# zrlhahaha/Direct12PBRRenderer

Measured on AMD Instinct MI355X. Metric: shaded Mpixel/s at 4K G-buffer (full deferred frame: clustered shade + bloom + auto-exposure + ACES), higher is better.
Workload: dtype f32

## Files before the change

direct12pbrrenderer_amd/csrc/bloom.hip:

```cpp
#include <type_traits>
#include "pbr_internal.hpp"
#include "pbr_device.hpp"

using namespace pbr;

__constant__ float c_gauss[9] = {0.0148f, 0.0459f, 0.1050f, 0.1941f, 0.2803f, 0.1941f, 0.1050f, 0.0459f, 0.0148f};

__device__ __forceinline__ float4 to4(F4 v) { return make_float4(v.x, v.y, v.z, v.w); }
__device__ __forceinline__ F4 from4(float4 v) { return f4(v.x, v.y, v.z, v.w); }

struct OutRect { int x0, y0, x1, y1, ox, oy, pitch; };
constexpr int PF_MAX_RECTS = 5;
struct OutRects {
    int n, ox, oy, pitch;
    int x0[PF_MAX_RECTS], y0[PF_MAX_RECTS], x1[PF_MAX_RECTS], y1[PF_MAX_RECTS], tiles_x[PF_MAX_RECTS], first[PF_MAX_RECTS + 1];
};
__global__ __launch_bounds__(256) void k_bloom_prefilter(const pbr_half* __restrict__ hdr, int w, int h, int pitch,
                                                           pbr_half* __restrict__ out, OutRect rc,
                                                           float tx, float ty, float threshold, float knee) {
    const int x = rc.x0 + blockIdx.x * 64 + threadIdx.x;
    const int y = rc.y0 + blockIdx.y * 4 + threadIdx.y;
    if (x >= rc.x1 || y >= rc.y1) return;
    const float u = (float)x * tx, v = (float)y * ty;
    const float ox[5] = {0.0f, -1.0f, -1.0f, 1.0f, 1.0f};
// ... 409 lines not shown
            constexpr int NR = PER_T / 2 + 2;
            const int base = (first >> 1) - 1 + (first & 1);
            V3 hrow[NR];
            const float wx0 = 1.0f - fx;
#pragma unroll
            for (int j = 0; j < NR; j++) {
                const H4* row = reinterpret_cast<const H4*>(in) + (size_t)min(base + j, ih - 1) * iw;
                const H4 c0 = row[ax0], c1 = row[ax1];
                hrow[j] = fma3(h3f(c1), fx, h3f(c0) * wx0);
            }
            auto blend = [&](auto parity) {
                constexpr int P = decltype(parity)::value;
#pragma unroll
                for (int k = 0; k < PER_T; k++) {
                    constexpr int dummy = 0; (void)dummy;
                    const int odd = (P + k) & 1;
                    const int i0 = (P + k + 1) / 2 - P;
                    const float fyk = odd ? 0.25f : 0.75f, wy0 = 1.0f - fyk;
                    const V3 r = fma3(hrow[i0 + 1], fyk, hrow[i0] * wy0);
                    smp[k] = make_float4(r.x, r.y, r.z, 0.0f);
                }
            };
            if (first & 1) blend(std::integral_constant<int, 1>{}); else blend(std::integral_constant<int, 0>{});
#pragma unroll
            for (int k = 0; k < PER_T; k++)
                if (DUAL) up[k] = reinterpret_cast<const H4*>(in2)[(size_t)(first + k) * ow + sx];
        } else {
            Tap2 taps[PER_T];
            float fy[PER_T];
#pragma unroll
            for (int k = 0; k < PER_T; k++) {
                const int jj = clampi(first + k, 0, oh - 1);
                int ay0, ay1;
                tap1d<MODE>(jj, ih, ay0, ay1, fy[k]);
                taps[k] = load_tap2<MODE>(in, iw, ax0, ax1, ay0, ay1);
                if (DUAL) up[k] = reinterpret_cast<const H4*>(in2)[(size_t)jj * ow + sx];
            }
#pragma unroll
            for (int k = 0; k < PER_T; k++) smp[k] = finish_tap2_rgb<MODE>(taps[k], fx, fy[k]);
        }
        if (has_halo) {
            const int jj = clampi(first + hk, 0, oh - 1);
            int ay0, ay1;
            tap1d<MODE>(jj, ih, ay0, ay1, hfy);
            htap = load_tap2<MODE>(in, iw, bx0, bx1, ay0, ay1);
            if (DUAL) hup = reinterpret_cast<const H4*>(in2)[(size_t)jj * ow + shx];
        }
#pragma unroll
        for (int k = 0; k < PER_T; k++) {
            line[lane] = smp[k];
            if (DUAL) line2[lane] = make_float4((float)up[k].x, (float)up[k].y, (float)up[k].z, 0.0f);
            if (has_halo && hk == k) {
                line[hc] = finish_tap2_rgb<MODE>(htap, hfx, hfy);
                if (DUAL) line2[hc] = make_float4((float)hup.x, (float)hup.y, (float)hup.z, 0.0f);
            }
            wave_sync();
            V3 g = gauss9_rgb(line + lane);
            if (DUAL) g = g + gauss9_rgb(line2 + lane);
            wave_sync();
            H4 th;
            th.x = to_half_rn(g.x); th.y = to_half_rn(g.y); th.z = to_half_rn(g.z); th.w = alpha_t;
            sT[r0 + k][lane] = th;
        }
    }
    __syncthreads();
#pragma unroll
    for (int k = 0; k < PER_O; k++) {
        const int r = wv + NW * k, y = y0 + r;
        if (x >= ow || y >= oh) continue;
        V3 a3 = v3(0.0f, 0.0f, 0.0f);
#pragma unroll
        for (int i = 0; i < 9; i++) a3 = fma3(h3f(sT[r + i][lane]), c_gauss[i], a3);
        const F4 a = f4(a3.x, a3.y, a3.z, alpha_v);
        if (TAIL == 0) {
            store_h4(out + 4 * ((size_t)y * out_pitch + x), a);
        } else {
            if (!(in_mx && y >= tr.my0 && y < tr.my1)) continue;
            const half4v a0 = round_h4(a);
            const F4 s = h4f(hdr_in[k]);
            H4 o;
            o.x = to_half_rn(s.x + (float)a0.x); o.y = to_half_rn(s.y + (float)a0.y); o.z = to_half_rn(s.z + (float)a0.z); o.w = to_half_rn(s.w + (float)a0.w);
            *reinterpret_cast<H4*>(out + 4 * ((size_t)(y - tr.by) * out_pitch + (x - tr.bx))) = o;
            if (TAIL == 2) {
                if (x >= tr.hx0 && x < tr.hx1 && y >= tr.hy0 && y < tr.hy1)
                    atomicAdd(&sh_hist[wv][luminance_bin_exact((float)o.x, (float)o.y, (float)o.z, min_log, inv_range)], 1u);
            }
        }
    }
    if (tile + (int)gridDim.x < n_tiles) __syncthreads();
    }
    if (TAIL == 2) {
        __syncthreads();
        for (int i = t; i < PBR_HISTOGRAM_BINS; i += NT) {
            uint32_t sum = 0;
#pragma unroll
            for (int w2 = 0; w2 < NW; w2++) sum += sh_hist[w2][i];
            if (sum) atomicAdd(&hist[i], sum);
        }
    }
}

__device__ __forceinline__ H4 ld_h4(const void* base, uint32_t byte_off) {
    return *reinterpret_cast<const H4*>(reinterpret_cast<const char*>(base) + byte_off);
}
__device__ __forceinline__ void gauss9_pair(const float2* e, float& ge, float& go) {
    const float s[10] = {e[0].x, e[0].y, e[1].x, e[1].y, e[2].x, e[2].y, e[3].x, e[3].y, e[4].x, e[4].y};
    float a = 0.0f, b = 0.0f;
#pragma unroll
    for (int i = 0; i < 9; i++) { a = __builtin_fmaf(s[i], c_gauss[i], a); b = __builtin_fmaf(s[i + 1], c_gauss[i], b); }
    ge = a; go = b;
}

namespace poly {
constexpr double G[9] = {0.0148, 0.0459, 0.1050, 0.1941, 0.2803, 0.1941, 0.1050, 0.0459, 0.0148};
constexpr double g(int k) { return (k < -4 || k > 4) ? 0.0 : G[k + 4]; }
constexpr float E(int j) { return (float)(0.75 * g(2 * j) + 0.25 * g(2 * j + 2) + 0.75 * g(2 * j + 1) + 0.25 * g(2 * j - 1)); }
}

template <bool DUAL, int TAIL, int TH, class VS = NoViews>
__global__ __launch_bounds__(512, 4) void k_blur_up_poly(const pbr_half* __restrict__ in_, int iw, int ih,
                                                          const pbr_half* __restrict__ in2_,
                                                          pbr_half* __restrict__ out_, int ow, int oh, int out_pitch_,
                                                          int tiles_x, int n_tiles,
                                                          TailRect tr, float min_log, float inv_range, VS vs,
                                                          uint32_t* __restrict__ hist_) {
    const pbr_half* __restrict__ in = in_;
    const pbr_half* __restrict__ in2 = in2_;
    pbr_half* __restrict__ out = out_;
    uint32_t* __restrict__ hist = hist_;
    int out_pitch = out_pitch_;
    if constexpr (!std::is_same_v<VS, NoViews>) {
        const int v = blockIdx.y;
        in = vs.in[v]; in2 = vs.in2[v]; out = vs.out[v]; hist = vs.hist[v]; out_pitch = vs.out_pitch[v];
    }
    constexpr int TW = 128, NP = TW / 2 + 4, NC = TW / 2 + 6, SR = TH + 8, NT = 512, NW = NT / 64;
    constexpr int NPAIR = TH / 2 + 5;
    constexpr int PPW = (NPAIR + NW - 1) / NW;
    constexpr int PER_O = TH / 4;
    static_assert(TH % 4 == 0 && (PPW + 1) * 6 <= 64 && 2 * PPW * 4 <= 64, "one halo entry per lane");
    __shared__ H4 sLineC[NW][NC + 2];
    __shared__ float2 sLineU[DUAL ? NW : 1][3][NP];
    __shared__ H4 sT[SR][TW];
    __shared__ uint32_t sh_hist[TAIL == 2 ? NW : 1][TAIL == 2 ? PBR_HISTOGRAM_BINS : 1];
    static_assert(sizeof(sLineC) + sizeof(sLineU) + sizeof(sT) + sizeof(sh_hist) <= 80 * 1024, "k_blur_up_poly: two blocks per CU no longer fit the LDS");
    const int t = threadIdx.x, lane = t & 63;
    const int wv = __builtin_amdgcn_readfirstlane(t >> 6);
    const int vc = t & 127, vg = __builtin_amdgcn_readfirstlane(t >> 7);
    if (TAIL == 2) {
        for (int i = t; i < NW * PBR_HISTOGRAM_BINS; i += NT) (&sh_hist[0][0])[i] = 0u;
    }
    const size_t a_at = (size_t)min(tr.my0 >> 1, ih - 1) * iw + min(tr.mx0 >> 1, iw - 1);
    float alpha_h = gauss9_const((float)reinterpret_cast<const H4*>(in)[a_at].w);
    if (DUAL) alpha_h = alpha_h + gauss9_const((float)reinterpret_cast<const H4*>(in2)[(size_t)min(tr.my0, oh - 1) * ow + min(tr.mx0, ow - 1)].w);
    const h16 alpha_t = to_half_rn(alpha_h);
    const float alpha_v = gauss9_const((float)alpha_t);
    const float a0w = (float)to_half_rn(alpha_v);
    auto wave_sync = [] {
        __builtin_amdgcn_fence(__ATOMIC_RELEASE, "wavefront");
        __builtin_amdgcn_wave_barrier();
        __builtin_amdgcn_fence(__ATOMIC_ACQUIRE, "wavefront");
    };
    for (int tile = blockIdx.x; tile < n_tiles; tile += gridDim.x) {
    const int x0 = (tr.tx0 + tile % tiles_x) * TW, y0 = (tr.ty0 + tile / tiles_x) * TH;
    const int xv = x0 + vc, rbase = vg * PER_O;
    H4 hdr_in[PER_O];
    const bool in_mx = TAIL != 0 && xv >= tr.mx0 && xv < tr.mx1;
    char* const hdr_row0 = reinterpret_cast<char*>(out) + (ptrdiff_t)(y0 + rbase - tr.by) * out_pitch * 8;
    const uint32_t hdr_x = (uint32_t)(xv - tr.bx) * 8u;
    const size_t hdr_pitch = (size_t)out_pitch * 8u;
    {
        const int i_first = wv * PPW;
        const int n_pairs = min(PPW, NPAIR - i_first);
        const int cb = (y0 >> 1) - 3 + i_first;
        const uint32_t ccol = (uint32_t)clampi((x0 >> 1) - 3 + lane, 0, iw - 1) * 8u;
        H4 cr[PPW + 1], chalo{};
        const int hk = lane / 6, hq = 64 + lane % 6;
        const bool has_halo = lane < 6 * (PPW + 1);
        H4 upE[DUAL ? 2 * PPW : 1], upO[DUAL ? 2 * PPW : 1], hupE{}, hupO{};
        const int uk = lane >> 2, uq = 64 + (lane & 3);
        const bool has_uhalo = DUAL && lane < 8 * PPW;
        if (n_pairs > 0) {
#pragma unroll
            for (int k = 0; k <= PPW; k++) {
                const char* row = reinterpret_cast<const char*>(in) + (size_t)clampi(cb + k, 0, ih - 1) * iw * 8u;
                cr[k] = ld_h4(row, ccol);
            }
            if (has_halo) {
                const char* row = reinterpret_cast<const char*>(in) + (size_t)clampi(cb + hk, 0, ih - 1) * iw * 8u;
                chalo = ld_h4(row, (uint32_t)clampi((x0 >> 1) - 3 + hq, 0, iw - 1) * 8u);
            }
            if (DUAL) {
                const int sxe = clampi(x0 - 4 + 2 * lane, 0, ow - 1), sxo = clampi(x0 - 3 + 2 * lane, 0, ow - 1);
#pragma unroll
                for (int k = 0; k < 2 * PPW; k++) {
                    const char* row = reinterpret_cast<const char*>(in2) + (size_t)clampi(y0 - 4 + 2 * i_first - 1 + k, 0, oh - 1) * ow * 8u;
                    upE[k] = ld_h4(row, (uint32_t)sxe * 8u); upO[k] = ld_h4(row, (uint32_t)sxo * 8u);
                }
                if (has_uhalo) {
                    const uint32_t row = (uint32_t)(clampi(y0 - 4 + 2 * i_first - 1 + uk, 0, oh - 1) * ow) * 8u;
                    hupE = ld_h4(in2, row + (uint32_t)clampi(x0 - 4 + 2 * uq, 0, ow - 1) * 8u); hupO = ld_h4(in2, row + (uint32_t)clampi(x0 - 3 + 2 * uq, 0, ow - 1) * 8u);
                }
            }
        }
        if (TAIL != 0) {
#pragma unroll
            for (int k = 0; k < PER_O; k++) {
                const int y = y0 + rbase + k;
                if (in_mx && y >= tr.my0 && y < tr.my1) hdr_in[k] = ld_h4(hdr_row0 + k * hdr_pitch, hdr_x);
            }
        }
        if (n_pairs > 0) {
            H4* line = sLineC[wv];
            float2 (*lineU)[NP] = sLineU[DUAL ? wv : 0];
            V3 pE = v3(0.0f, 0.0f, 0.0f), pO = pE;
#pragma unroll
            for (int k = 0; k <= PPW; k++) {
                if (k > n_pairs) break;
                line[lane] = cr[k];
                if (has_halo && hk == k) line[hq] = chalo;
                wave_sync();
                V3 e[7];
#pragma unroll
                for (int j = 0; j < 7; j++) e[j] = h3f(line[lane + j]);
                wave_sync();
                constexpr float PE[6] = {poly::E(-3), poly::E(-2), poly::E(-1), poly::E(0), poly::E(1), poly::E(2)};
                V3 cE = v3(0.0f, 0.0f, 0.0f), cO = cE;
#pragma unroll
                for (int j = 0; j < 6; j++) { cE = fma3(e[j], PE[j], cE); cO = fma3(e[j + 1], PE[5 - j], cO); }
                if (k > 0) {
#pragma unroll
                    for (int half = 0; half < 2; half++) {
                        const int r = 2 * (i_first + k - 1) - 1 + half;
                        if (r < 0 || r >= SR) continue;
                        const float fy = half ? 0.75f : 0.25f, wy0 = 1.0f - fy;
                        V3 bE = fma3(cE, fy, pE * wy0), bO = fma3(cO, fy, pO * wy0);
                        if (DUAL) {
                            const int u = 2 * (k - 1) + half;
                            lineU[0][lane] = make_float2((float)upE[u].x, (float)upO[u].x); lineU[1][lane] = make_float2((float)upE[u].y, (float)upO[u].y);
                            lineU[2][lane] = make_float2((float)upE[u].z, (float)upO[u].z);
                            if (has_uhalo && uk == u) {
                                lineU[0][uq] = make_float2((float)hupE.x, (float)hupO.x); lineU[1][uq] = make_float2((float)hupE.y, (float)hupO.y);
                                lineU[2][uq] = make_float2((float)hupE.z, (float)hupO.z);
                            }
                            wave_sync();
                            V3 uE, uO;
                            gauss9_pair(lineU[0] + lane, uE.x, uO.x); gauss9_pair(lineU[1] + lane, uE.y, uO.y); gauss9_pair(lineU[2] + lane, uE.z, uO.z);
                            wave_sync();
                            bE = bE + uE; bO = bO + uO;
                        }
                        struct alignas(16) H8 { H4 a, b; } th;
                        th.a.x = to_half_rn(bE.x); th.a.y = to_half_rn(bE.y); th.a.z = to_half_rn(bE.z); th.a.w = alpha_t;
                        th.b.x = to_half_rn(bO.x); th.b.y = to_half_rn(bO.y); th.b.z = to_half_rn(bO.z); th.b.w = alpha_t;
                        *reinterpret_cast<H8*>(&sT[r][2 * lane]) = th;
                    }
                }
                pE = cE; pO = cO;
            }
        }
    }
    __syncthreads();
    {
        H4 win[PER_O + 8];
#pragma unroll
        for (int i = 0; i < PER_O + 8; i++) win[i] = sT[rbase + i][vc];
#pragma unroll
        for (int k = 0; k < PER_O; k++) {
            const int y = y0 + rbase + k;
            if (xv >= ow || y >= oh) continue;
            V3 a3 = v3(0.0f, 0.0f, 0.0f);
#pragma unroll
            for (int i = 0; i < 9; i++) a3 = fma3(h3f(win[k + i]), c_gauss[i], a3);
            const F4 a = f4(a3.x, a3.y, a3.z, alpha_v);
            if (TAIL == 0) {
                store_h4(out + 4 * ((size_t)y * out_pitch + xv), a);
            } else {
                if (!(in_mx && y >= tr.my0 && y < tr.my1)) continue;
                const half2v a01 = round_h2(a3.x, a3.y);
                const h16 a2 = to_half_rn(a3.z);
                const F4 s = h4f(hdr_in[k]);
                struct alignas(8) O4 { half2v lo, hi; } o;
                o.lo = round_h2(s.x + (float)a01.x, s.y + (float)a01.y);
                o.hi = round_h2(s.z + (float)a2, s.w + a0w);
                *reinterpret_cast<O4*>(hdr_row0 + k * hdr_pitch + hdr_x) = o;
                if (TAIL == 2) {
                    if (xv >= tr.hx0 && xv < tr.hx1 && y >= tr.hy0 && y < tr.hy1)
                        atomicAdd(&sh_hist[wv][luminance_bin_exact((float)o.lo.x, (float)o.lo.y, (float)o.hi.x, min_log, inv_range)], 1u);
                }
            }
        }
    }
    if (tile + (int)gridDim.x < n_tiles) __syncthreads();
    }
    if (TAIL == 2) {
        __syncthreads();
        for (int i = t; i < PBR_HISTOGRAM_BINS; i += NT) {
            uint32_t sum = 0;
#pragma unroll
            for (int w2 = 0; w2 < NW; w2++) sum += sh_hist[w2][i];
            if (sum) atomicAdd(&hist[i], sum);
        }
    }
}

static int blur_h_rows(uint32_t ow, uint32_t oh) {
    const uint64_t row_blocks = (uint64_t)((ow + 255) / 256) * oh;
    int rows = (int)(row_blocks / 2048);
    return rows < 1 ? 1 : (rows > HB_MAX_ROWS ? HB_MAX_ROWS : rows);
}

static bool exact_half(uint32_t n) { return (n & 1u) == 0u && n <= 8192u; }

template <int MODE, bool DUAL, int TAIL, bool MV = false>
static pbr_status launch_hv(pbr_ctx* ctx, const LevelViews& lv, uint32_t nv, uint32_t iw, uint32_t ih, uint32_t ow, uint32_t oh,
                            const uint32_t* rect, float min_log, float inv_range,
                            const uint32_t* merge_rect = nullptr, const uint32_t* buf_origin = nullptr) {
    using VS = std::conditional_t<MV, LevelViews, NoViews>;
    VS vs{};
    if constexpr (MV) vs = lv;
    const pbr_half* in = MV ? nullptr : lv.in[0];
    const pbr_half* in2 = MV ? nullptr : lv.in2[0];
    pbr_half* out = MV ? nullptr : lv.out[0];
    uint32_t* hist = MV ? nullptr : lv.hist[0];
    const int out_pitch = MV ? 0 : lv.out_pitch[0];
    TailRect tr;
    tr.hx0 = rect ? (int)rect[0] : 0; tr.hy0 = rect ? (int)rect[1] : 0;
    tr.hx1 = rect ? (int)(rect[0] + rect[2]) : 0; tr.hy1 = rect ? (int)(rect[1] + rect[3]) : 0;
    tr.mx0 = merge_rect ? (int)merge_rect[0] : 0; tr.my0 = merge_rect ? (int)merge_rect[1] : 0;
    tr.mx1 = merge_rect ? (int)(merge_rect[0] + merge_rect[2]) : (int)ow; tr.my1 = merge_rect ? (int)(merge_rect[1] + merge_rect[3]) : (int)oh;
    tr.bx = buf_origin ? (int)buf_origin[0] : 0; tr.by = buf_origin ? (int)buf_origin[1] : 0;
    static const int hist_blocks = pbr::knob_int("PBR_BLOOM_HIST_BLOCKS", 1024);
    auto even_blocks = [nv](int n_tiles) { const int per = (n_tiles * (int)nv + hist_blocks - 1) / hist_blocks; return (n_tiles + per - 1) / per; };
    if constexpr (MODE == M_UP) {
        static const int wide_forced = pbr::knob_int("PBR_BLOOM_WIDE", -1);
        const int wtx0 = tr.mx0 / 128, wty0 = tr.my0 / 32;
        const int wtiles_x = (tr.mx1 + 127) / 128 - wtx0, wn = wtiles_x * ((tr.my1 + 31) / 32 - wty0);
        if (wide_forced >= 0 ? wide_forced == 1 : (wn >= 400 && !ctx->bloom_shader_order)) {
            tr.tx0 = wtx0; tr.ty0 = wty0;
            const int wb = TAIL == 2 ? even_blocks(wn) : wn;
            hipLaunchKernelGGL((k_blur_up_poly<DUAL, TAIL, 32, VS>), dim3(wb, nv), dim3(512), 0, ctx->stream,
                               in, (int)iw, (int)ih, in2, out, (int)ow, (int)oh, out_pitch, wtiles_x, wn, tr, min_log, inv_range, vs, hist);
            return launched(ctx, MV ? "k_blur_up_poly<views>" : "k_blur_up_poly");
        }
    }
    const bool big = (uint64_t)((tr.mx1 + 63) / 64 - tr.mx0 / 64) * ((tr.my1 + 31) / 32 - tr.my0 / 32) >= 900;
    const int th = big ? 32 : 16;
    tr.tx0 = tr.mx0 / 64; tr.ty0 = tr.my0 / th;
    const int tiles_x = (tr.mx1 + 63) / 64 - tr.tx0;
    const int n_tiles = tiles_x * ((tr.my1 + th - 1) / th - tr.ty0);
    const int blocks = TAIL == 2 ? even_blocks(n_tiles) : n_tiles;
    if (big) {
        hipLaunchKernelGGL((k_blur_hv<MODE, DUAL, TAIL, 32, 512, VS>), dim3(blocks, nv), dim3(512), 0, ctx->stream,
                           in, (int)iw, (int)ih, in2, out, (int)ow, (int)oh, out_pitch, tiles_x, n_tiles, tr, min_log, inv_range, vs, hist);
    } else {
        hipLaunchKernelGGL((k_blur_hv<MODE, DUAL, TAIL, 16, 512, VS>), dim3(blocks, nv), dim3(512), 0, ctx->stream,
                           in, (int)iw, (int)ih, in2, out, (int)ow, (int)oh, out_pitch, tiles_x, n_tiles, tr, min_log, inv_range, vs, hist);
    }
    return launched(ctx, MV ? "k_blur_hv<views>" : "k_blur_hv");
}

static OutRects out_rects(const OutRect* rcs, int n) {
    OutRects rs{};
    rs.n = n; rs.ox = rcs[0].ox; rs.oy = rcs[0].oy; rs.pitch = rcs[0].pitch;
    int blocks = 0;
    for (int r = 0; r < n; r++) {
        rs.x0[r] = rcs[r].x0; rs.y0[r] = rcs[r].y0; rs.x1[r] = rcs[r].x1; rs.y1[r] = rcs[r].y1;
        rs.tiles_x[r] = (rcs[r].x1 - rcs[r].x0 + PF_TW - 1) / PF_TW;
        rs.first[r] = blocks;
        blocks += rs.tiles_x[r] * ((rcs[r].y1 - rcs[r].y0 + PF_TH - 1) / PF_TH);
    }
    rs.first[n] = blocks;
    return rs;
}

extern "C" {

static pbr_status prefilter_launch(pbr_ctx* ctx, const pbr_half* hdr, uint32_t w, uint32_t h, uint32_t pitch,
                                   pbr_half* out, const OutRect* rcs, int n, float threshold, float knee) {
    const uint32_t ow = w >> 1, oh = h >> 1;
    const float tx = 1.0f / (float)ow, ty = 1.0f / (float)oh;
    if (exact_half(w) && exact_half(h)) {
        const OutRects rs = out_rects(rcs, n);
        hipLaunchKernelGGL(k_bloom_prefilter_2x<NoViews>, dim3(rs.first[n]), dim3(256), 0, ctx->stream, hdr, (int)w, (int)h, (int)pitch, NoViews{}, out, rs, threshold, knee);
        return launched(ctx, "k_bloom_prefilter_2x");
    }
    for (int r = 0; r < n; r++) {
        const uint32_t rw = (uint32_t)(rcs[r].x1 - rcs[r].x0), rh = (uint32_t)(rcs[r].y1 - rcs[r].y0);
        dim3 grid((rw + 63) / 64, (rh + 3) / 4);
        hipLaunchKernelGGL(k_bloom_prefilter, grid, dim3(64, 4), 0, ctx->stream, hdr, (int)w, (int)h, (int)pitch, out, rcs[r], tx, ty, threshold, knee);
        pbr_status st = launched(ctx, "k_bloom_prefilter");
        if (st) return st;
    }
    return PBR_OK;
}

pbr_status pbr_bloom_prefilter(pbr_ctx* ctx, const pbr_half* hdr, uint32_t w, uint32_t h, uint32_t pitch,
                               pbr_half* out, float threshold, float knee) {
    if (!ctx) return PBR_ERR_INVALID;
    PBR_REQUIRE(ctx, hdr && out, "pbr_bloom_prefilter: null pointer");
    PBR_REQUIRE(ctx, (w >> 1) >= 1 && (h >> 1) >= 1 && w <= 65535 && h <= 65535 && pitch >= w, "pbr_bloom_prefilter: bad size");
    const OutRect rc{0, 0, (int)(w >> 1), (int)(h >> 1), 0, 0, (int)(w >> 1)};
    return prefilter_launch(ctx, hdr, w, h, pitch, out, &rc, 1, threshold, knee);
}

pbr_status pbr_bloom_prefilter_rect(pbr_ctx* ctx, const pbr_half* hdr, uint32_t w, uint32_t h, uint32_t pitch,
                                    pbr_half* out, uint32_t out_pitch, uint32_t out_x, uint32_t out_y,
                                    const uint32_t rect[4], float threshold, float knee) {
    if (!ctx) return PBR_ERR_INVALID;
    PBR_REQUIRE(ctx, hdr && out && rect, "pbr_bloom_prefilter_rect: null pointer");
    PBR_REQUIRE(ctx, (w >> 1) >= 1 && (h >> 1) >= 1 && w <= 65535 && h <= 65535 && pitch >= w, "pbr_bloom_prefilter_rect: bad size");
    PBR_REQUIRE(ctx, rect[2] >= 1 && rect[3] >= 1 && rect[0] + rect[2] <= (w >> 1) && rect[1] + rect[3] <= (h >> 1), "pbr_bloom_prefilter_rect: rect outside the half-res image");
    PBR_REQUIRE(ctx, out_pitch >= out_x + rect[0] + rect[2] && out_pitch <= 65535 && out_y <= 65535, "pbr_bloom_prefilter_rect: rect does not fit the output pitch");
    const OutRect rc{(int)rect[0], (int)rect[1], (int)(rect[0] + rect[2]), (int)(rect[1] + rect[3]), (int)out_x, (int)out_y, (int)out_pitch};
    return prefilter_launch(ctx, hdr, w, h, pitch, out, &rc, 1, threshold, knee);
}

pbr_status pbr_bloom_prefilter_rects(pbr_ctx* ctx, const pbr_half* hdr, uint32_t w, uint32_t h, uint32_t pitch,
                                     pbr_half* out, uint32_t out_pitch, uint32_t out_x, uint32_t out_y,
                                     const uint32_t (*rects)[4], uint32_t n_rects, float threshold, float knee) {
    if (!ctx) return PBR_ERR_INVALID;
    PBR_REQUIRE(ctx, hdr && out && rects && n_rects >= 1 && n_rects <= (uint32_t)PF_MAX_RECTS, "pbr_bloom_prefilter_rects: null pointer / 1 .. 5 rectangles");
    PBR_REQUIRE(ctx, (w >> 1) >= 1 && (h >> 1) >= 1 && w <= 65535 && h <= 65535 && pitch >= w && out_pitch <= 65535 && out_y <= 65535, "pbr_bloom_prefilter_rects: bad size");
    OutRect rcs[PF_MAX_RECTS];
    for (uint32_t r = 0; r < n_rects; r++) {
        const uint32_t* q = rects[r];
        PBR_REQUIRE(ctx, q[2] >= 1 && q[3] >= 1 && q[0] + q[2] <= (w >> 1) && q[1] + q[3] <= (h >> 1) && out_pitch >= out_x + q[0] + q[2],
                    "pbr_bloom_prefilter_rects: rectangle outside the half-res image / the output pitch");
        rcs[r] = OutRect{(int)q[0], (int)q[1], (int)(q[0] + q[2]), (int)(q[1] + q[3]), (int)out_x, (int)out_y, (int)out_pitch};
    }
    return prefilter_launch(ctx, hdr, w, h, pitch, out, rcs, (int)n_rects, threshold, knee);
}

pbr_status pbr_blur_h(pbr_ctx* ctx, const pbr_half* in, uint32_t iw, uint32_t ih, pbr_half* out, uint32_t ow, uint32_t oh) {
    if (!ctx) return PBR_ERR_INVALID;
    PBR_REQUIRE(ctx, in && out, "pbr_blur_h: null pointer");
    PBR_REQUIRE(ctx, iw && ih && ow && oh && iw <= 65535 && ih <= 65535 && ow <= 65535 && oh <= 65535, "pbr_blur_h: bad size");
    const float tx = 1.0f / (float)ow, ty = 1.0f / (float)oh;
    const int rows = blur_h_rows(ow, oh);
    dim3 grid((ow + 255) / 256, (oh + rows - 1) / rows);
    hipLaunchKernelGGL(k_blur_h<false>, grid, dim3(256), 0, ctx->stream, in, (int)iw, (int)ih, (const pbr_half*)nullptr, 0, 0, out, (int)ow, (int)oh, tx, ty, rows);
    return launched(ctx, "k_blur_h");
}

pbr_status pbr_blur_v(pbr_ctx* ctx, const pbr_half* in, uint32_t iw, uint32_t ih, pbr_half* out, uint32_t ow, uint32_t oh) {
    if (!ctx) return PBR_ERR_INVALID;
    PBR_REQUIRE(ctx, in && out, "pbr_blur_v: null pointer");
    PBR_REQUIRE(ctx, iw && ih && ow && oh && iw <= 65535 && ih <= 65535 && ow <= 65535 && oh <= 65535, "pbr_blur_v: bad size");
    const float tx = 1.0f / (float)ow, ty = 1.0f / (float)oh;
    dim3 grid((ow + VT_W - 1) / VT_W, (oh + VT_R - 1) / VT_R);
    hipLaunchKernelGGL(k_blur_v, grid, dim3(VT_W, 4), 0, ctx->stream, in, (int)iw, (int)ih, out, (int)ow, (int)oh, tx, ty);
    return launched(ctx, "k_blur_v");
}

pbr_status pbr_bloom_upsample_add(pbr_ctx* ctx, const pbr_half* upper, uint32_t uw, uint32_t uh,
                                  const pbr_half* lower, uint32_t lw, uint32_t lh, pbr_half* out) {
    if (!ctx) return PBR_ERR_INVALID;
    PBR_REQUIRE(ctx, upper && lower && out, "pbr_bloom_upsample_add: null pointer");
    PBR_REQUIRE(ctx, uw && uh && lw && lh && uw <= 65535 && uh <= 65535, "pbr_bloom_upsample_add: bad size");
    const float tx = 1.0f / (float)uw, ty = 1.0f / (float)uh;
    const int rows = blur_h_rows(uw, uh);
    dim3 grid((uw + 255) / 256, (uh + rows - 1) / rows);
    hipLaunchKernelGGL(k_blur_h<true>, grid, dim3(256), 0, ctx->stream, lower, (int)lw, (int)lh, upper, (int)uw, (int)uh, out, (int)uw, (int)uh, tx, ty, rows);
    return launched(ctx, "k_blur_h<dual>");
}

pbr_status pbr_bloom_merge(pbr_ctx* ctx, pbr_half* hdr, uint32_t pitch, const pbr_half* in, uint32_t w, uint32_t h) {
    if (!ctx) return PBR_ERR_INVALID;
    PBR_REQUIRE(ctx, hdr && in, "pbr_bloom_merge: null pointer");
    PBR_REQUIRE(ctx, w && h && w <= 65535 && h <= 65535 && pitch >= w, "pbr_bloom_merge: bad size");
    dim3 grid((w + 255) / 256, h);
    hipLaunchKernelGGL(k_bloom_merge, grid, dim3(256), 0, ctx->stream, hdr, (int)pitch, in, (int)w, (int)h);
    return launched(ctx, "k_bloom_merge");
}

pbr_status pbr_bloom_up_level(pbr_ctx* ctx, const pbr_half* upper, const pbr_half* lower, uint32_t lw, uint32_t lh,
                              pbr_half* out, uint32_t ow, uint32_t oh) {
    if (!ctx) return PBR_ERR_INVALID;
    PBR_REQUIRE(ctx, lower && out && out != lower && out != upper, "pbr_bloom_up_level: null pointer / out aliases an input");
    PBR_REQUIRE(ctx, lw >= 1 && lh >= 1 && ow == 2 * lw && oh == 2 * lh && exact_half(ow) && exact_half(oh), "pbr_bloom_up_level: out must be exactly twice lower, even, <= 8192");
    LevelViews lv{};
    lv.in[0] = lower; lv.in2[0] = upper; lv.out[0] = out; lv.out_pitch[0] = (int)ow;
    if (upper) return launch_hv<M_UP, true, 0>(ctx, lv, 1, lw, lh, ow, oh, nullptr, 0.0f, 0.0f);
    return launch_hv<M_UP, false, 0>(ctx, lv, 1, lw, lh, ow, oh, nullptr, 0.0f, 0.0f);
}

static pbr_status bloom_final(pbr_ctx* ctx, const pbr_half* b0, pbr_half* hdr, uint32_t w, uint32_t h, uint32_t pitch,
                              const uint32_t* hist_rect, float min_log, float inv_range, uint32_t* hist256) {
    const float tx = 1.0f / (float)w, ty = 1.0f / (float)h;
    const int tiles_x = (int)((w + VT_W - 1) / VT_W), tiles_y = (int)((h + VT_R - 1) / VT_R);
    int blocks = tiles_x * tiles_y;
    if (blocks > 1280) blocks = 1280;
    if (hist256) {
        hipLaunchKernelGGL(k_blur_v_merge<true>, dim3(blocks), dim3(VT_W, 4), 0, ctx->stream, b0, (int)w, (int)h, tx, ty, hdr, (int)pitch, tiles_x, tiles_y,
                           (int)hist_rect[0], (int)hist_rect[1], (int)(hist_rect[0] + hist_rect[2]), (int)(hist_rect[1] + hist_rect[3]), min_log, inv_range, hist256);
    } else {
        hipLaunchKernelGGL(k_blur_v_merge<false>, dim3(blocks), dim3(VT_W, 4), 0, ctx->stream, b0, (int)w, (int)h, tx, ty, hdr, (int)pitch, tiles_x, tiles_y,
                           0, 0, 0, 0, 0.0f, 0.0f, (uint32_t*)nullptr);
    }
    return launched(ctx, "k_blur_v_merge");
}

}

struct BloomView { pbr_half* hdr; uint32_t pitch; pbr_half* A; pbr_half* B; uint32_t* hist; };

template <bool MV>
static pbr_status bloom_pass(pbr_ctx* ctx, const BloomView* v, uint32_t n, uint32_t w, uint32_t h, bool prefilter, float threshold, float knee,
                             const uint32_t* hist_rect, float min_log, float inv_range, const uint32_t* merge0 = nullptr, const uint32_t* origin = nullptr) {
    auto W = [&](uint32_t l) { return w >> l; };
    auto H = [&](uint32_t l) { return h >> l; };
    auto off = [&](uint32_t l) { return (size_t)4 * pbr_bloom_level_offset(w, h, l); };
    auto exact = [&](uint32_t l) { return exact_half(W(l)) && exact_half(H(l)); };
    pbr_status r;
    if (prefilter) {
        const OutRect whole{0, 0, (int)W(1), (int)H(1), 0, 0, (int)W(1)};
        if (MV && exact(0)) {
            PrefilterViews pv{};
            for (uint32_t i = 0; i < n; i++) { pv.hdr[i] = v[i].hdr; pv.out[i] = v[i].A + off(1); pv.pitch[i] = (int)v[i].pitch; }
            const OutRects rs = out_rects(&whole, 1);
            hipLaunchKernelGGL(k_bloom_prefilter_2x<PrefilterViews>, dim3(rs.first[1], n), dim3(256), 0, ctx->stream,
                               nullptr, (int)w, (int)h, 0, pv, nullptr, rs, threshold, knee);
            if ((r = launched(ctx, "k_bloom_prefilter_2x<views>"))) return r;
        } else {
            for (uint32_t i = 0; i < n; i++)
                if ((r = prefilter_launch(ctx, v[i].hdr, w, h, v[i].pitch, v[i].A + off(1), &whole, 1, threshold, knee))) return r;
        }
    }
    for (uint32_t k = 0; k < PBR_BLOOM_STEP; k++) {
        const uint32_t up = k + 1, lo = k + 2;
        if (exact(up)) {
            LevelViews lv{};
            for (uint32_t i = 0; i < n; i++) { lv.in[i] = v[i].A + off(up); lv.out[i] = v[i].A + off(lo); lv.out_pitch[i] = (int)W(lo); }
            if ((r = launch_hv<M_DOWN, false, 0, MV>(ctx, lv, n, W(up), H(up), W(lo), H(lo), nullptr, 0.0f, 0.0f))) return r;
        } else {
            for (uint32_t i = 0; i < n; i++) {
                if ((r = pbr_blur_h(ctx, v[i].A + off(up), W(up), H(up), v[i].B + off(lo), W(lo), H(lo)))) return r;
                if ((r = pbr_blur_v(ctx, v[i].B + off(lo), W(lo), H(lo), v[i].A + off(lo), W(lo), H(lo)))) return r;
            }
        }
    }
    uint32_t need[PBR_BLOOM_MIPS][4];
    static const bool shrink = pbr::knob_int("PBR_BLOOM_SHRINK", 1) != 0;
    const bool use_need = merge0 != nullptr && shrink;
    if (use_need) {
        int x0 = (int)merge0[0], y0 = (int)merge0[1], x1 = (int)(merge0[0] + merge0[2]), y1 = (int)(merge0[1] + merge0[3]);
        for (uint32_t l = 1; l < PBR_BLOOM_MIPS; l++) {
            x0 = (x0 - 4) / 2 - 2; y0 = (y0 - 4) / 2 - 2; x1 = (x1 + 4 + 1) / 2 + 2; y1 = (y1 + 4 + 1) / 2 + 2;
            const int cx0 = x0 < 0 ? 0 : x0, cy0 = y0 < 0 ? 0 : y0, cx1 = x1 > (int)W(l) ? (int)W(l) : x1, cy1 = y1 > (int)H(l) ? (int)H(l) : y1;
            need[l][0] = (uint32_t)cx0; need[l][1] = (uint32_t)cy0; need[l][2] = (uint32_t)(cx1 - cx0); need[l][3] = (uint32_t)(cy1 - cy0);
            x0 = cx0; y0 = cy0; x1 = cx1; y1 = cy1;
        }
    }
    bool res_in_b = false;
    uint32_t res_level = PBR_BLOOM_MIPS - 1;
    auto res = [&](uint32_t i) { return (const pbr_half*)(res_in_b ? v[i].B : v[i].A) + off(res_level); };
    for (int k = PBR_BLOOM_STEP - 1; k >= 0; k--) {
        const uint32_t up = (uint32_t)k + 1;
        if (exact(up)) {
            LevelViews lv{};
            for (uint32_t i = 0; i < n; i++) { lv.in[i] = res(i); lv.in2[i] = v[i].A + off(up); lv.out[i] = v[i].B + off(up); lv.out_pitch[i] = (int)W(up); }
            if ((r = launch_hv<M_UP, true, 0, MV>(ctx, lv, n, W(up + 1), H(up + 1), W(up), H(up), nullptr, 0.0f, 0.0f,
                                                  use_need ? need[up] : nullptr))) return r;
            res_in_b = true;
        } else {
            for (uint32_t i = 0; i < n; i++) {
                if ((r = pbr_bloom_upsample_add(ctx, v[i].A + off(up), W(up), H(up), res(i), W(up + 1), H(up + 1), v[i].B + off(up)))) return r;
                if ((r = pbr_blur_v(ctx, v[i].B + off(up), W(up), H(up), v[i].A + off(up), W(up), H(up)))) return r;
            }
            res_in_b = false;
        }
        res_level = up;
    }
    if (exact(0)) {
        LevelViews lv{};
        for (uint32_t i = 0; i < n; i++) { lv.in[i] = res(i); lv.out[i] = v[i].hdr; lv.out_pitch[i] = (int)v[i].pitch; lv.hist[i] = v[i].hist; }
        if constexpr (!MV)
            if (!v[0].hist) return launch_hv<M_UP, false, 1>(ctx, lv, 1, w >> 1, h >> 1, w, h, nullptr, 0.0f, 0.0f, merge0, origin);
        return launch_hv<M_UP, false, 2, MV>(ctx, lv, n, w >> 1, h >> 1, w, h, hist_rect, min_log, inv_range, merge0, origin);
    }
    for (uint32_t i = 0; i < n; i++) {
        if ((r = pbr_blur_h(ctx, res(i), w >> 1, h >> 1, v[i].B, w, h))) return r;
        if ((r = bloom_final(ctx, v[i].B, v[i].hdr, w, h, v[i].pitch, hist_rect, min_log, inv_range, v[i].hist))) return r;
    }
    return PBR_OK;
}

extern "C" {

static pbr_status bloom_impl(pbr_ctx* ctx, pbr_half* hdr, uint32_t w, uint32_t h, uint32_t pitch, pbr_half* A, pbr_half* B,
                             float threshold, float knee, const uint32_t* hist_rect, float min_log, float inv_range, uint32_t* hist256) {
    PBR_REQUIRE(ctx, hdr && A && B, "pbr_bloom: null pointer");
    PBR_REQUIRE(ctx, (w >> (PBR_BLOOM_MIPS - 1)) >= 1 && (h >> (PBR_BLOOM_MIPS - 1)) >= 1, "pbr_bloom: image too small for 5 mips");
    PBR_REQUIRE(ctx, w <= 65535 && h <= 65535 && pitch >= w, "pbr_bloom: bad size");
    const BloomView v{hdr, pitch, A, B, hist256};
    return bloom_pass<false>(ctx, &v, 1, w, h, true, threshold, knee, hist_rect, min_log, inv_range);
}

pbr_status pbr_bloom(pbr_ctx* ctx, pbr_half* hdr, uint32_t w, uint32_t h, uint32_t pitch,
                     pbr_half* A, pbr_half* B, float threshold, float knee) {
    if (!ctx) return PBR_ERR_INVALID;
    return bloom_impl(ctx, hdr, w, h, pitch, A, B, threshold, knee, nullptr, 0.0f, 0.0f, nullptr);
}

pbr_status pbr_bloom_histogram(pbr_ctx* ctx, pbr_half* hdr, uint32_t w, uint32_t h, uint32_t pitch,
                               pbr_half* A, pbr_half* B, float threshold, float knee,
                               const uint32_t rect[4], float min_log, float inv_range, uint32_t* hist256) {
    if (!ctx) return PBR_ERR_INVALID;
    PBR_REQUIRE(ctx, rect && hist256, "pbr_bloom_histogram: null pointer");
    PBR_REQUIRE(ctx, rect[2] >= 1 && rect[3] >= 1 && rect[0] + rect[2] <= w && rect[1] + rect[3] <= h, "pbr_bloom_histogram: rect outside the image");
    return bloom_impl(ctx, hdr, w, h, pitch, A, B, threshold, knee, rect, min_log, inv_range, hist256);
}

pbr_status pbr_bloom_histogram_views(pbr_ctx* ctx, const pbr_view* views, uint32_t n, uint32_t w, uint32_t h,
                                     float threshold, float knee, float min_log, float inv_range) {
    if (!ctx) return PBR_ERR_INVALID;
    PBR_REQUIRE(ctx, views_count_ok(views, n), "pbr_bloom_histogram_views: need 1 .. PBR_MAX_VIEWS views");
    PBR_REQUIRE(ctx, (w >> (PBR_BLOOM_MIPS - 1)) >= 1 && (h >> (PBR_BLOOM_MIPS - 1)) >= 1, "pbr_bloom_histogram_views: image too small for 5 mips");
    PBR_REQUIRE(ctx, w <= 65535 && h <= 65535, "pbr_bloom_histogram_views: bad size");
    BloomView bv[PBR_MAX_VIEWS];
    for (uint32_t i = 0; i < n; i++) {
        const pbr_view& v = views[i];
        PBR_REQUIRE(ctx, v.hdr && v.chain_a && v.chain_b && v.hist256, "pbr_bloom_histogram_views: null pointer");
        PBR_REQUIRE(ctx, v.hdr_pitch >= w, "pbr_bloom_histogram_views: bad size");
        bv[i] = BloomView{v.hdr, v.hdr_pitch, v.chain_a, v.chain_b, v.hist256};
    }
    const size_t chain_bytes = pbr_bloom_chain_texels(w, h) * 8u;
    PBR_REQUIRE(ctx, views_disjoint(views, n, 4, [&](const pbr_view& v, int k, uintptr_t& lo, uintptr_t& hi) {
                    if (k == 0) { lo = addr(v.hdr); hi = lo + ((size_t)v.hdr_pitch * (h - 1) + w) * 8u; }
                    else if (k == 1) { lo = addr(v.chain_a); hi = lo + chain_bytes; }
                    else if (k == 2) { lo = addr(v.chain_b); hi = lo + chain_bytes; }
                    else { lo = addr(v.hist256); hi = lo + PBR_HISTOGRAM_BINS * sizeof(uint32_t); } }),
                "pbr_bloom_histogram_views: two views share an HDR target, a bloom chain or a histogram");
    const uint32_t rect[4] = {0, 0, w, h};
    return bloom_pass<true>(ctx, bv, n, w, h, true, threshold, knee, rect, min_log, inv_range);
}

pbr_status pbr_bloom_tiled(pbr_ctx* ctx, pbr_half* hdr, uint32_t hdr_pitch, const uint32_t hdr_rect[4],
                           uint32_t ew, uint32_t eh, pbr_half* A, pbr_half* B, const uint32_t merge_rect[4],
                           float min_log, float inv_range, uint32_t* hist256) {
    if (!ctx) return PBR_ERR_INVALID;
// ... 16 lines not shown
```

Before: 17550.

## Add wave-streaming bloom upsample kernel with sliding-window vertical blur

Adds k_blur_up_stream, where each wavefront owns a 128-pixel-wide column strip and walks down a vertical segment. It keeps a 16-row register window for the vertical 9-tap gaussian, uses per-wave LDS lines for the horizontal filters, and double-buffers global loads across steps. This replaces tile-based blocks whose vertical halos are re-read and need block-wide barriers, using only wave-level syncs instead. It is enabled by default for the histogram-tail and dual non-tail large upsample passes. In exchange it carries heavy register pressure and segment-boundary halo overhead.

After: 17270. 0.984x the previous value.

```diff
diff --git a/direct12pbrrenderer_amd/csrc/bloom.hip b/direct12pbrrenderer_amd/csrc/bloom.hip
--- a/direct12pbrrenderer_amd/csrc/bloom.hip
+++ b/direct12pbrrenderer_amd/csrc/bloom.hip
@@ -735,6 +735,213 @@
     }
 }
 
+constexpr int STREAM_NW = 4;
+constexpr int STREAM_DEFAULT = 3;
+template <bool DUAL, int TAIL, class VS = NoViews>
+__global__ __launch_bounds__(64 * STREAM_NW, 2) void k_blur_up_stream(const pbr_half* __restrict__ in_, int iw, int ih,
+                                                                       const pbr_half* __restrict__ in2_,
+                                                                       pbr_half* __restrict__ out_, int ow, int oh, int out_pitch_,
+                                                                       int n_strips, int n_tasks, int seg,
+                                                                       TailRect tr, float min_log, float inv_range, VS vs,
+                                                                       uint32_t* __restrict__ hist_) {
+    const pbr_half* __restrict__ in = in_;
+    const pbr_half* __restrict__ in2 = in2_;
+    pbr_half* __restrict__ out = out_;
+    uint32_t* __restrict__ hist = hist_;
+    int out_pitch = out_pitch_;
+    if constexpr (!std::is_same_v<VS, NoViews>) {
+        const int v = blockIdx.y;
+        in = vs.in[v]; in2 = vs.in2[v]; out = vs.out[v]; hist = vs.hist[v]; out_pitch = vs.out_pitch[v];
+    }
+    constexpr int NW = STREAM_NW, NT = 64 * NW, NP = 64 + 4, NC = 64 + 6;
+    __shared__ H4 sLineC[NW][NC + 2];
+    __shared__ float2 sLineU[DUAL ? NW : 1][3][NP];
+    __shared__ uint32_t sh_hist[TAIL == 2 ? NW : 1][TAIL == 2 ? PBR_HISTOGRAM_BINS : 1];
+    static_assert(sizeof(sLineC) + sizeof(sLineU) + sizeof(sh_hist) <= 80 * 1024, "k_blur_up_stream: two blocks per CU no longer fit the LDS");
+    const int t = threadIdx.x, lane = t & 63;
+    const int wv = __builtin_amdgcn_readfirstlane(t >> 6);
+    auto wave_sync = [] {
+        __builtin_amdgcn_fence(__ATOMIC_RELEASE, "wavefront");
+        __builtin_amdgcn_wave_barrier();
+        __builtin_amdgcn_fence(__ATOMIC_ACQUIRE, "wavefront");
+    };
+    if (TAIL == 2) {
+        for (int i = lane; i < PBR_HISTOGRAM_BINS; i += 64) sh_hist[wv][i] = 0u;
+        wave_sync();
+    }
+    const int task = __builtin_amdgcn_readfirstlane((int)blockIdx.x * NW + wv);
+    if (task < n_tasks) {
+    float alpha_h = gauss9_const((float)reinterpret_cast<const H4*>(in)[0].w);
+    if (DUAL) alpha_h = alpha_h + gauss9_const((float)reinterpret_cast<const H4*>(in2)[0].w);
+    const h16 alpha_t = to_half_rn(alpha_h);
+    const float alpha_v = gauss9_const((float)alpha_t);
+    const float a0w = (float)to_half_rn(alpha_v);
+    const int x0 = (task % n_strips) * 128, sg = task / n_strips;
+    const int Ys = sg * seg - 1, Ye = min(Ys + seg, oh);
+    const int n_steps = (Ye - Ys + 7) / 8 + 1;
+    const int m0 = (Ys - 5) / 2;
+    const int xv = x0 + 2 * lane;
+    const bool in_x = xv < ow;
+    struct alignas(8) H8 { H4 a, b; };
+    struct alignas(8) O4 { half2v lo, hi; };
+    struct alignas(8) O8 { O4 a, b; };
+    const uint32_t ccol = (uint32_t)clampi((x0 >> 1) - 3 + lane, 0, iw - 1) * 8u;
+    const int hk = lane / 6, hq = 64 + lane % 6;
+    const bool has_halo = lane < 24;
+    const uint32_t hcol = (uint32_t)clampi((x0 >> 1) - 3 + hq, 0, iw - 1) * 8u;
+    const int uk = lane >> 2, uq = 64 + (lane & 3);
+    const bool has_uhalo = DUAL && lane < 32;
+    const uint32_t sxe = (uint32_t)clampi(x0 - 4 + 2 * lane, 0, ow - 1) * 8u, sxo = (uint32_t)clampi(x0 - 3 + 2 * lane, 0, ow - 1) * 8u;
+    const uint32_t hxe = (uint32_t)clampi(x0 - 4 + 2 * uq, 0, ow - 1) * 8u, hxo = (uint32_t)clampi(x0 - 3 + 2 * uq, 0, ow - 1) * 8u;
+    const size_t hdr_pitch = (size_t)out_pitch * 8u;
+    char* const hdr_col = reinterpret_cast<char*>(out) + (size_t)xv * 8u;
+    auto row_ok = [&](int y) { return y >= 0 && y >= Ys && y < Ye; };
+    auto coarse_row = [&](int m) { return reinterpret_cast<const char*>(in) + (size_t)clampi(m, 0, ih - 1) * iw * 8u; };
+    auto fine_row = [&](int f) { return reinterpret_cast<const char*>(in2) + (size_t)clampi(f, 0, oh - 1) * ow * 8u; };
+
+    struct Step {
+        H4 cr[4], chalo;
+        H4 upE[DUAL ? 8 : 1], upO[DUAL ? 8 : 1], hupE, hupO;
+        H8 hdr[TAIL != 0 ? 8 : 1];
+    };
+    auto load_step = [&](Step& L, int c) {
+        const int m1 = m0 + 1 + 4 * c, fc = Ys - 4 + 8 * c;
+#pragma unroll
+        for (int k = 0; k < 4; k++) L.cr[k] = ld_h4(coarse_row(m1 + k), ccol);
+        if (has_halo) L.chalo = ld_h4(coarse_row(m1 + hk), hcol);
+        if (DUAL) {
+#pragma unroll
+            for (int k = 0; k < 8; k++) { const char* row = fine_row(fc + k); L.upE[k] = ld_h4(row, sxe); L.upO[k] = ld_h4(row, sxo); }
+            if (has_uhalo) { const char* row = fine_row(fc + uk); L.hupE = ld_h4(row, hxe); L.hupO = ld_h4(row, hxo); }
+        }
+        if (TAIL != 0) {
+#pragma unroll
+            for (int k = 0; k < 8; k++) {
+                const int y = fc - 4 + k;
+                if (in_x && c > 0 && row_ok(y)) L.hdr[k] = *reinterpret_cast<const H8*>(hdr_col + (size_t)y * hdr_pitch);
+            }
+        }
+    };
+    H4* line = sLineC[wv];
+    float2 (*lineU)[NP] = sLineU[DUAL ? wv : 0];
+    constexpr float PE[6] = {poly::E(-3), poly::E(-2), poly::E(-1), poly::E(0), poly::E(1), poly::E(2)};
+    auto filter_line = [&](V3& cE, V3& cO) {
+        wave_sync();
+        V3 e[7];
+#pragma unroll
+        for (int j = 0; j < 7; j++) e[j] = h3f(line[lane + j]);
+        wave_sync();
+        cE = v3(0.0f, 0.0f, 0.0f); cO = cE;
+#pragma unroll
+        for (int j = 0; j < 6; j++) { cE = fma3(e[j], PE[j], cE); cO = fma3(e[j + 1], PE[5 - j], cO); }
+    };
+    V3 pE, pO;
+    {
+        const char* row = coarse_row(m0);
+        const H4 c0 = ld_h4(row, ccol);
+        H4 h0{};
+        if (lane < 6) h0 = ld_h4(row, hcol);
+        line[lane] = c0;
+        if (lane < 6) line[hq] = h0;
+        filter_line(pE, pO);
+    }
+    H8 win[16];
+#pragma unroll
+    for (int i = 0; i < 16; i++) win[i] = H8{};
+    auto run_step = [&](const Step& L, int c) {
+        const int fc = Ys - 4 + 8 * c;
+#pragma unroll
+        for (int k = 0; k < 4; k++) {
+            line[lane] = L.cr[k];
+            if (has_halo && hk == k) line[hq] = L.chalo;
+            V3 cE, cO;
+            filter_line(cE, cO);
+#pragma unroll
+            for (int half = 0; half < 2; half++) {
+                const float fy = half ? 0.75f : 0.25f, wy0 = 1.0f - fy;
+                V3 bE = fma3(cE, fy, pE * wy0), bO = fma3(cO, fy, pO * wy0);
+                if (DUAL) {
+                    const int u = 2 * k + half;
+                    lineU[0][lane] = make_float2((float)L.upE[u].x, (float)L.upO[u].x); lineU[1][lane] = make_float2((float)L.upE[u].y, (float)L.upO[u].y);
+                    lineU[2][lane] = make_float2((float)L.upE[u].z, (float)L.upO[u].z);
+                    if (has_uhalo && uk == u) {
+                        lineU[0][uq] = make_float2((float)L.hupE.x, (float)L.hupO.x); lineU[1][uq] = make_float2((float)L.hupE.y, (float)L.hupO.y);
+                        lineU[2][uq] = make_float2((float)L.hupE.z, (float)L.hupO.z);
+                    }
+                    wave_sync();
+                    V3 uE, uO;
+                    gauss9_pair(lineU[0] + lane, uE.x, uO.x); gauss9_pair(lineU[1] + lane, uE.y, uO.y); gauss9_pair(lineU[2] + lane, uE.z, uO.z);
+                    wave_sync();
+                    bE = bE + uE; bO = bO + uO;
+                }
+                H8 th;
+                th.a.x = to_half_rn(bE.x); th.a.y = to_half_rn(bE.y); th.a.z = to_half_rn(bE.z); th.a.w = alpha_t;
+                th.b.x = to_half_rn(bO.x); th.b.y = to_half_rn(bO.y); th.b.z = to_half_rn(bO.z); th.b.w = alpha_t;
+                win[8 + 2 * k + half] = th;
+            }
+            pE = cE; pO = cO;
+        }
+        if (c > 0 && in_x) {
+#pragma unroll
+            for (int k = 0; k < 8; k++) {
+                const int y = fc - 4 + k;
+                if (!row_ok(y)) continue;
+                V3 a3 = v3(0.0f, 0.0f, 0.0f), b3 = a3;
+#pragma unroll
+                for (int i = 0; i < 9; i++) { a3 = fma3(h3f(win[k + i].a), c_gauss[i], a3); b3 = fma3(h3f(win[k + i].b), c_gauss[i], b3); }
+                if (TAIL == 0) {
+                    const half4v ha = round_h4(f4(a3.x, a3.y, a3.z, alpha_v)), hb = round_h4(f4(b3.x, b3.y, b3.z, alpha_v));
+                    struct alignas(8) S8 { half4v a, b; } st{ha, hb};
+                    *reinterpret_cast<S8*>(hdr_col + (size_t)y * hdr_pitch) = st;
+                } else {
+                    auto merge = [&](const V3& g, const H4& hdr_in) {
+                        const half2v a01 = round_h2(g.x, g.y);
+                        const h16 a2 = to_half_rn(g.z);
+                        const F4 s = h4f(hdr_in);
+                        O4 o;
+                        o.lo = round_h2(s.x + (float)a01.x, s.y + (float)a01.y);
+                        o.hi = round_h2(s.z + (float)a2, s.w + a0w);
+                        return o;
+                    };
+                    O8 o;
+                    o.a = merge(a3, L.hdr[k].a); o.b = merge(b3, L.hdr[k].b);
+                    *reinterpret_cast<O8*>(hdr_col + (size_t)y * hdr_pitch) = o;
+                    if (TAIL == 2) {
+                        if (y >= tr.hy0 && y < tr.hy1) {
+                            if (xv >= tr.hx0 && xv < tr.hx1)
+                                atomicAdd(&sh_hist[wv][luminance_bin_exact((float)o.a.lo.x, (float)o.a.lo.y, (float)o.a.hi.x, min_log, inv_range)], 1u);
+                            if (xv + 1 >= tr.hx0 && xv + 1 < tr.hx1)
+                                atomicAdd(&sh_hist[wv][luminance_bin_exact((float)o.b.lo.x, (float)o.b.lo.y, (float)o.b.hi.x, min_log, inv_range)], 1u);
+                        }
+                    }
+                }
+            }
+        }
+#pragma unroll
+        for (int i = 0; i < 8; i++) win[i] = win[i + 8];
+    };
+    Step sa, sb;
+    load_step(sa, 0);
+    for (int c = 0; c < n_steps; c += 2) {
+        load_step(sb, c + 1);
+        run_step(sa, c);
+        if (c + 1 < n_steps) {
+            load_step(sa, c + 2);
+            run_step(sb, c + 1);
+        }
+    }
+    }
+    if (TAIL == 2) {
+        __syncthreads();
+        for (int i = t; i < PBR_HISTOGRAM_BINS; i += NT) {
+            uint32_t sum = 0;
+#pragma unroll
+            for (int w2 = 0; w2 < NW; w2++) sum += sh_hist[w2][i];
+            if (sum) atomicAdd(&hist[i], sum);
+        }
+    }
+}
+
 static int blur_h_rows(uint32_t ow, uint32_t oh) {
     const uint64_t row_blocks = (uint64_t)((ow + 255) / 256) * oh;
     int rows = (int)(row_blocks / 2048);
@@ -768,6 +975,24 @@
         const int wtx0 = tr.mx0 / 128, wty0 = tr.my0 / 32;
         const int wtiles_x = (tr.mx1 + 127) / 128 - wtx0, wn = wtiles_x * ((tr.my1 + 31) / 32 - wty0);
         if (wide_forced >= 0 ? wide_forced == 1 : (wn >= 400 && !ctx->bloom_shader_order)) {
+            static const int stream_mask = pbr::knob_int("PBR_BLOOM_STREAM", STREAM_DEFAULT);
+            constexpr int stream_bit = TAIL == 2 ? 1 : (TAIL == 0 && DUAL) ? 2 : 0;
+            if constexpr (stream_bit != 0) {
+                if ((stream_mask & stream_bit) && !merge_rect && !buf_origin) {
+                    static const int wps = pbr::knob_int("PBR_BLOOM_STREAM_WPS", 2), seg_forced = pbr::knob_int("PBR_BLOOM_STREAM_SEG", 0);
+                    const int cus = ctx->cu_count > 0 ? ctx->cu_count : 256;
+                    const int slots = cus * 4 * wps / (int)nv > 0 ? cus * 4 * wps / (int)nv : 1;
+                    const int n_strips = ((int)ow + 127) / 128;
+                    int seg = (int)(((uint64_t)(oh + 1) * n_strips + slots - 1) / slots);
+                    seg = (seg + 7) / 8 * 8;
+                    seg = seg < 16 ? 16 : (seg > 128 ? 128 : seg);
+                    if (seg_forced > 0) seg = (seg_forced + 7) / 8 * 8;
+                    const int n_tasks = n_strips * (((int)oh + 1 + seg - 1) / seg);
+                    hipLaunchKernelGGL((k_blur_up_stream<DUAL, TAIL, VS>), dim3((n_tasks + STREAM_NW - 1) / STREAM_NW, nv), dim3(64 * STREAM_NW), 0, ctx->stream,
+                                       in, (int)iw, (int)ih, in2, out, (int)ow, (int)oh, out_pitch, n_strips, n_tasks, seg, tr, min_log, inv_range, vs, hist);
+                    return launched(ctx, MV ? "k_blur_up_stream<views>" : "k_blur_up_stream");
+                }
+            }
             tr.tx0 = wtx0; tr.ty0 = wty0;
             const int wb = TAIL == 2 ? even_blocks(wn) : wn;
             hipLaunchKernelGGL((k_blur_up_poly<DUAL, TAIL, 32, VS>), dim3(wb, nv), dim3(512), 0, ctx->stream,
```
